# Abolfazlmsl/Oriented-Object-Detection

Measured on AMD Instinct MI355X. Metric: 416px tiles/sec (whole node), YOLOv11n-OBB 3ch, higher is better.
Workload: dtype f32; 1 GPU; YOLOv11n-OBB 3ch 416x416 tiled inference, single-scale (BASELINE configs[1]): forward + decode + ProbIoU NMS + border filter + per-tile merge + final polygon-IoU merge; step_pipelining=True, nc=12, weights=synthetic seeded, cls bias -8 (no checkpoint offline), final_detections=12170

## Files before the change

oriented-object-detection_amd/csrc/c3k2f32.h:

```cpp
#pragma once
#include <hip/hip_runtime.h>

#include <vector>

#include "conv.h"

namespace obb {

struct C3k2F32Launch {
    TensorRef cat;
    TensorRef out;
    const float *w1 = nullptr, *w2 = nullptr, *wc = nullptr;
    const float *b1 = nullptr, *b2 = nullptr, *bc = nullptr;
    int B = 0, H = 0, W = 0, C = 16, CO = 64;
};

bool c3k2f32_supported(int C, int CO, int H, int W);
std::vector<int> c3k2f32_cout_perm(int CO);
void c3k2f32_tile(int H, int W, int &TH, int &TW);
hipError_t launch_c3k2f32(const C3k2F32Launch &L, hipStream_t st);

}
```

oriented-object-detection_amd/csrc/c3k2f32.hip:

```cpp
#include "c3k2f32.h"

#include <algorithm>
#include <mutex>

namespace obb {

typedef __attribute__((ext_vector_type(4))) float f32x4;
typedef __attribute__((ext_vector_type(4))) unsigned int u32x4;

struct C3k2Params {
    const float *cat; int64_t cat_bs; int cat_cs, cat_co; unsigned cat_span;
    float *out; int64_t out_bs; int out_cs, out_co, out_blk, out_ps;
    const float *wall, *b1, *b2;
    int H, W, TH, TW, tiles_x, tiles_y;
    float inv_xw, inv_tw2, inv_tw;
};

__device__ __forceinline__ float silu32c(float x) { return x * __builtin_amdgcn_rcpf(1.0f + __expf(-x)); }

constexpr int kC3MaxX = 448, kC3MaxT = 324;

template <int C, int CO>
__global__ __launch_bounds__(512, 4) void k_c3k2_f32(const C3k2Params P) {
    extern __shared__ __attribute__((aligned(16))) char smem[];
    constexpr int NT = 512, CH = C / 2, PSTX = C * 4 + 16, PSTT = CH * 4 + 16;
    constexpr int CPK1 = C / 4, KP1 = 9 * CPK1 / 4, CPK2 = CH / 4, KP2 = (9 * CPK2) / 4, KR2 = (9 * CPK2) % 4, KPC = 3 * C / 16, NFC = CO / 16;
    static_assert((9 * CPK1) % 4 == 0, "conv 1: whole pieces only");
    constexpr int XOFF = 0, TOFF = kC3MaxX * PSTX, W1OFF = TOFF + kC3MaxT * PSTT, W2OFF = W1OFF + KP1 * 1024, WCOFF = W2OFF + KP2 * 1024 + KR2 * 256,
                  BCOFF = WCOFF + NFC * KPC * 1024, NWCH = (BCOFF + CO * 4 - W1OFF) / 16;
    constexpr int F1 = 3, F2 = 2;
    constexpr unsigned NOPIX = 0xffffffffu;
    const int tid = threadIdx.x, lane = tid & 63, wave = __builtin_amdgcn_readfirstlane(tid >> 6), g = lane >> 4, pl = lane & 15;
    const int t = blockIdx.x, tx_i = t % P.tiles_x, r_ = t / P.tiles_x, ty_i = r_ % P.tiles_y, b = r_ / P.tiles_y;
    const int oy0 = ty_i * P.TH, ox0 = tx_i * P.TW;
    const int XW = P.TW + 4, XH = P.TH + 4, TW2 = P.TW + 2, TH2 = P.TH + 2;
    const int npix1 = TH2 * TW2, npix2 = P.TH * P.TW;

    const __amdgpu_buffer_rsrc_t cat_rsrc = __builtin_amdgcn_make_buffer_rsrc((void *)(P.cat + (int64_t)b * P.cat_bs + P.cat_co), 0, (int)P.cat_span, 0x00020000);
    const __amdgpu_buffer_rsrc_t w_rsrc = __builtin_amdgcn_make_buffer_rsrc((void *)P.wall, 0, NWCH * 16, 0x00020000);
    constexpr int MAXLD = (kC3MaxX * CPK1 + NT - 1) / NT, MAXW = (NWCH + NT - 1) / NT;
    u32x4 xr[MAXLD], wr[MAXW];
    const int nchunkX = XH * XW * CPK1;
#pragma unroll
    for (int k = 0; k < MAXLD; ++k) {
        const int idx = tid + k * NT, pix = idx / CPK1, c = idx - pix * CPK1;
        const int iy = (int)(((float)pix + 0.5f) * P.inv_xw), ix = pix - iy * XW;
        const int gy = oy0 - 2 + iy, gx = ox0 - 2 + ix;
        const bool ok = idx < nchunkX && gy >= 0 && gy < P.H && gx >= 0 && gx < P.W;
        xr[k] = __builtin_amdgcn_raw_buffer_load_b128(cat_rsrc, ok ? (unsigned)((((int64_t)gy * P.W + gx) * P.cat_cs + C + c * 4) * 4) : NOPIX, 0, 0);
    }
#pragma unroll
    for (int k = 0; k < MAXW; ++k) wr[k] = __builtin_amdgcn_raw_buffer_load_b128(w_rsrc, (unsigned)min(tid + k * NT, NWCH - 1) * 16u, 0, 0);
    const int nfrag1 = (npix1 + 15) >> 4, nfrag2 = (npix2 + 15) >> 4;
    f32x4 y0v[F2];
    int opix[F2];
    int xc[F2], tb[F2];
#pragma unroll
    for (int i = 0; i < F2; ++i) {
        const int p0 = (wave + 8 * i) * 16 + pl, p = min(p0, npix2 - 1);
        const int r = (int)(((float)p + 0.5f) * P.inv_tw), x = p - r * P.TW;
        const int oy = oy0 + r, ox = ox0 + x;
        const bool ok = p0 < npix2 && oy < P.H && ox < P.W;
        opix[i] = ok ? oy * P.W + ox : -1;
        y0v[i] = __builtin_bit_cast(f32x4, __builtin_amdgcn_raw_buffer_load_b128(cat_rsrc, ok ? (unsigned)(((int64_t)opix[i] * P.cat_cs + g * 4) * 4) : NOPIX, 0, 0));
        xc[i] = ((r + 2) * XW + x + 2) * PSTX;
        tb[i] = (r * TW2 + x) * PSTT;
    }
#pragma unroll
    for (int k = 0; k < MAXLD; ++k) {
        const int idx = tid + k * NT, pix = idx / CPK1, c = idx - pix * CPK1;
        if (idx < nchunkX) *reinterpret_cast<u32x4 *>(smem + XOFF + pix * PSTX + c * 16) = xr[k];
    }
#pragma unroll
    for (int k = 0; k < MAXW; ++k) {
        const int idx = tid + k * NT;
        if (idx < NWCH) *reinterpret_cast<u32x4 *>(smem + W1OFF + idx * 16) = wr[k];
    }
    __syncthreads();

    {
        int xb[F1];
        bool val[F1];
#pragma unroll
        for (int i = 0; i < F1; ++i) {
            const int f = wave + 8 * i;
            val[i] = f < nfrag1;
            const int p = min(f * 16 + pl, npix1 - 1);
            const int r = (int)(((float)p + 0.5f) * P.inv_tw2), x = p - r * TW2;
            xb[i] = (r * XW + x) * PSTX;
        }
        f32x4 acc[F1];
#pragma unroll
        for (int i = 0; i < F1; ++i) acc[i] = f32x4{0.f, 0.f, 0.f, 0.f};
        for (int piece = 0; piece < KP1; ++piece) {
            const f32x4 w = *reinterpret_cast<const f32x4 *>(smem + W1OFF + piece * 1024 + lane * 16);
            const int q = piece * 4 + g, tap = q / CPK1, c0 = q - tap * CPK1, dy = (tap * 11) >> 5, dx = tap - dy * 3;
            const int off = (dy * XW + dx) * PSTX + c0 * 16;
            f32x4 a[F1];
#pragma unroll
            for (int i = 0; i < F1; ++i) a[i] = *reinterpret_cast<const f32x4 *>(smem + XOFF + xb[i] + off);
#pragma unroll
            for (int s = 0; s < 4; ++s)
#pragma unroll
                for (int i = 0; i < F1; ++i)
                    if (val[i]) acc[i] = __builtin_amdgcn_mfma_f32_16x16x4f32(w[s], a[i][s], acc[i], 0, 0, 0);
        }
        const float4 bv = *reinterpret_cast<const float4 *>(P.b1 + 4 * g);
#pragma unroll
        for (int i = 0; i < F1; ++i) {
            const int p = (wave + 8 * i) * 16 + pl;
            if (!val[i] || p >= npix1 || 4 * g >= CH) continue;
            const int r = (int)(((float)p + 0.5f) * P.inv_tw2), x = p - r * TW2;
            const int gy = oy0 - 1 + r, gx = ox0 - 1 + x;
            const bool inside = gy >= 0 && gy < P.H && gx >= 0 && gx < P.W;
            float4 o = make_float4(0.f, 0.f, 0.f, 0.f);
            if (inside) o = make_float4(silu32c(acc[i][0] + bv.x), silu32c(acc[i][1] + bv.y), silu32c(acc[i][2] + bv.z), silu32c(acc[i][3] + bv.w));
            *reinterpret_cast<float4 *>(smem + TOFF + (r * TW2 + x) * PSTT + g * 16) = o;
        }
    }
    __syncthreads();

    bool val2[F2];
#pragma unroll
    for (int i = 0; i < F2; ++i) val2[i] = wave + 8 * i < nfrag2;
    f32x4 acc2[F2];
#pragma unroll
    for (int i = 0; i < F2; ++i) acc2[i] = f32x4{0.f, 0.f, 0.f, 0.f};
#pragma unroll
    for (int piece = 0; piece < KP2; ++piece) {
        const f32x4 w = *reinterpret_cast<const f32x4 *>(smem + W2OFF + piece * 1024 + lane * 16);
        const int q = piece * 4 + g, tap = q / CPK2, c0 = q - tap * CPK2, dy = (tap * 11) >> 5, dx = tap - dy * 3;
        const int off = (dy * TW2 + dx) * PSTT + c0 * 16;
        f32x4 a[F2];
#pragma unroll
        for (int i = 0; i < F2; ++i) a[i] = *reinterpret_cast<const f32x4 *>(smem + TOFF + tb[i] + off);
#pragma unroll
        for (int s = 0; s < 4; ++s)
#pragma unroll
            for (int i = 0; i < F2; ++i)
                if (val2[i]) acc2[i] = __builtin_amdgcn_mfma_f32_16x16x4f32(w[s], a[i][s], acc2[i], 0, 0, 0);
    }
#pragma unroll
    for (int rr = 0; rr < KR2; ++rr) {
        const float w1 = *reinterpret_cast<const float *>(smem + W2OFF + KP2 * 1024 + rr * 256 + lane * 4);
        const int q = KP2 * 4 + rr, tap = q / CPK2, c0 = q - tap * CPK2, dy = (tap * 11) >> 5, dx = tap - dy * 3;
        const int off = (dy * TW2 + dx) * PSTT + c0 * 16 + g * 4;
#pragma unroll
        for (int i = 0; i < F2; ++i) {
            const float a1 = *reinterpret_cast<const float *>(smem + TOFF + tb[i] + off);
            if (val2[i]) acc2[i] = __builtin_amdgcn_mfma_f32_16x16x4f32(w1, a1, acc2[i], 0, 0, 0);
        }
    }
    f32x4 y1v[F2], y2v[F2];
    {
        const float4 bv = *reinterpret_cast<const float4 *>(P.b2 + 4 * g);
#pragma unroll
        for (int i = 0; i < F2; ++i) {
            y1v[i] = *reinterpret_cast<const f32x4 *>(smem + XOFF + xc[i] + g * 16);
            y2v[i][0] = y1v[i][0] + silu32c(acc2[i][0] + bv.x); y2v[i][1] = y1v[i][1] + silu32c(acc2[i][1] + bv.y);
            y2v[i][2] = y1v[i][2] + silu32c(acc2[i][2] + bv.z); y2v[i][3] = y1v[i][3] + silu32c(acc2[i][3] + bv.w);
        }
    }

    f32x4 acc3[F2][NFC];
#pragma unroll
    for (int i = 0; i < F2; ++i)
#pragma unroll
        for (int nf = 0; nf < NFC; ++nf) acc3[i][nf] = f32x4{0.f, 0.f, 0.f, 0.f};
#pragma unroll
    for (int piece = 0; piece < KPC; ++piece) {
        f32x4 bop[F2];
#pragma unroll
        for (int i = 0; i < F2; ++i) bop[i] = piece == 0 ? y0v[i] : (piece == 1 ? y1v[i] : y2v[i]);
#pragma unroll
        for (int nf = 0; nf < NFC; ++nf) {
            const f32x4 w = *reinterpret_cast<const f32x4 *>(smem + WCOFF + (nf * KPC + piece) * 1024 + lane * 16);
#pragma unroll
            for (int s = 0; s < 4; ++s)
#pragma unroll
                for (int i = 0; i < F2; ++i)
                    if (val2[i]) acc3[i][nf] = __builtin_amdgcn_mfma_f32_16x16x4f32(w[s], bop[i][s], acc3[i][nf], 0, 0, 0);
        }
    }
#pragma unroll
    for (int i = 0; i < F2; ++i) {
        if (!val2[i] || opix[i] < 0) continue;
        const int ca = P.out_co + 16 * g;
        float *op = P.out + (int64_t)b * P.out_bs + (int64_t)opix[i] * P.out_cs + (P.out_blk ? (int64_t)(ca >> 3) * P.out_ps + (ca & 7) : (int64_t)ca);
#pragma unroll
        for (int nf = 0; nf < NFC; ++nf) {
            const float4 bv = *reinterpret_cast<const float4 *>(smem + BCOFF + (nf * 16 + 4 * g) * 4);
            const float4 o = make_float4(silu32c(acc3[i][nf][0] + bv.x), silu32c(acc3[i][nf][1] + bv.y), silu32c(acc3[i][nf][2] + bv.z), silu32c(acc3[i][nf][3] + bv.w));
            float *o4 = P.out_blk ? op + (int64_t)(nf >> 1) * P.out_ps + 4 * (nf & 1) : op + 4 * nf;
            *reinterpret_cast<float4 *>(o4) = o;
        }
    }
}

void c3k2f32_tile(int H, int W, int &TH, int &TW) {
    TW = std::min(W, 52);
    if (W > 52 && W % 52 && W % 2 == 0 && W / 2 <= 52) TW = W / 2;
    int th = 1;
    while (th + 1 <= H && (th + 5) * (TW + 4) <= kC3MaxX && (th + 3) * (TW + 2) <= kC3MaxT && (th + 3) * (TW + 2) <= 24 * 16 && (th + 1) * TW <= 16 * 16) ++th;
    TH = th;
}

bool c3k2f32_supported(int C, int CO, int H, int W) {
    if (C != 16 || CO != 64 || H < 1 || W < 1) return false;
    int TH, TW;
    c3k2f32_tile(H, W, TH, TW);
    return (TH + 4) * (TW + 4) <= kC3MaxX && (TH + 2) * (TW + 2) <= kC3MaxT && (TH + 2) * (TW + 2) <= 24 * 16 && TH * TW <= 16 * 16;
}

std::vector<int> c3k2f32_cout_perm(int CO) {
    std::vector<int> p(CO);
    for (int f = 0; f < CO / 16; ++f)
        for (int r = 0; r < 16; ++r) p[16 * f + r] = 16 * (r >> 2) + 4 * f + (r & 3);
    return p;
}

hipError_t launch_c3k2f32(const C3k2F32Launch &L, hipStream_t st) {
    if (!c3k2f32_supported(L.C, L.CO, L.H, L.W) || L.cat.cpb || (L.cat.cs & 3) || (L.cat.co & 3) || !L.w1 || !L.b1 || !L.b2 || L.B < 1) return hipErrorInvalidValue;
    if (L.out.cpb && !(L.out.cpb == 2 && L.out.cs == 8 && L.out.co % 8 == 0 && L.out.ps > 0)) return hipErrorInvalidValue;
    if (!L.out.cpb && ((L.out.cs | L.out.co) & 3)) return hipErrorInvalidValue;
    C3k2Params P;
    P.cat = (const float *)L.cat.p; P.cat_bs = L.cat.bs; P.cat_cs = L.cat.cs; P.cat_co = L.cat.co;
    const int64_t span = ((int64_t)L.H * L.W * L.cat.cs - L.cat.co) * 4;
    if (span <= 0 || span >= (1ll << 32) - 65536) return hipErrorInvalidValue;
    P.cat_span = (unsigned)span;
    P.out = (float *)L.out.p; P.out_bs = L.out.bs; P.out_cs = L.out.cs; P.out_co = L.out.co; P.out_blk = L.out.cpb ? 1 : 0; P.out_ps = (int)L.out.ps;
    P.wall = L.w1; P.b1 = L.b1; P.b2 = L.b2;
    P.H = L.H; P.W = L.W;
    c3k2f32_tile(L.H, L.W, P.TH, P.TW);
    P.tiles_x = (L.W + P.TW - 1) / P.TW; P.tiles_y = (L.H + P.TH - 1) / P.TH;
    P.inv_xw = 1.0f / (float)(P.TW + 4); P.inv_tw2 = 1.0f / (float)(P.TW + 2); P.inv_tw = 1.0f / (float)P.TW;
    const int64_t ntiles = (int64_t)L.B * P.tiles_y * P.tiles_x;
    if (ntiles >= (1ll << 31)) return hipErrorInvalidValue;
    constexpr int C = 16, CO = 64;
    constexpr size_t lds = (size_t)kC3MaxX * (C * 4 + 16) + (size_t)kC3MaxT * (C / 2 * 4 + 16) + 9 * 1024 + (4 * 1024 + 2 * 256) + (CO / 16) * 3 * 1024 + CO * 4;
    static std::once_flag once;
    static hipError_t attr_err = hipSuccess;
    std::call_once(once, [] { attr_err = hipFuncSetAttribute((const void *)k_c3k2_f32<16, 64>, hipFuncAttributeMaxDynamicSharedMemorySize, 80 * 1024); });
    if (attr_err != hipSuccess) return attr_err;
    hipLaunchKernelGGL((k_c3k2_f32<16, 64>), dim3((unsigned)ntiles), dim3(512), lds, st, P);
    return hipGetLastError();
}

}
```

oriented-object-detection_amd/csrc/engine.hip:

```cpp
#include <algorithm>
#include <cmath>
#include <cstdlib>
#include <cstring>
#include <map>
#include <memory>
#include <string>
#include <tuple>

#include "bneck.h"
#include "c3k2f32.h"
#include "c3kimg.h"
#include "ctx.h"
#include "dwpw.h"
#include "f32path.h"
#include "front.h"
#include "nnops.h"
#include "pw32.h"
#include "stem.h"

namespace obb {

static constexpr int kRegMax = 16;

struct ConvRecord {
// ... 551 lines not shown
            st.second.assign(a->b, a->b + a->c2);
            st.second.insert(st.second.end(), b->b, b->b + b->c2);
            ConvRecord r = *a;
            r.name = nm; r.c2 = a->c2 + b->c2; r.w = st.first.data(); r.b = st.second.data();
            M.recs[nm] = r;
        }
        return nm;
    }

    bool bottleneck(const std::string &name, Slice in, int H, int W, Slice out, double e, const char *cv2name = nullptr, Slice y0 = Slice(),
                    Slice cv2out = Slice()) {
        int c_ = (int)(out.C * e);
        if (M.bneck && in.buf >= 0 && in.buf == out.buf && P.bufs[in.buf].blk == in.C && in.C == out.C && c_ * 2 == in.C &&
            bneck_supported(in.C, H, W)) {
            const ConvRecord *r1 = rec(name + ".cv1"), *r2 = rec(name + ".cv2");
            if (!r1 || !r2 || err) return false;
            if (r1->k == 3 && r2->k == 3 && r1->s == 1 && r2->s == 1 && r1->g == 1 && r2->g == 1 && r1->act && r2->act && r1->c1 == in.C &&
                r1->c2 == c_ && r2->c1 == c_ && r2->c2 == in.C) {
                Op op;
                op.type = OP_BNECK; op.name = name; op.in = in; op.out = out; op.H = H; op.W = W; op.Ho = H; op.Wo = W;
                BneckLaunch &L = op.bneck;
                L.H = H; L.W = W; L.C = in.C; L.f16 = M.f16;
                ConvTiling t1{1, 1, 1, 1, in.C}, t2{1, 1, 1, in.C / 16, c_};
                L.w1pk = upload(pack_conv_weights(r1->w, c_, in.C, 3, t1, nullptr, 0, M.f16));
                L.w2pk = upload(pack_conv_weights(r2->w, in.C, c_, 3, t2, nullptr, 0, M.f16));
                std::vector<float> b1(128, 0.f), b2(128, 0.f);
                for (int c = 0; c < c_; ++c) b1[c] = r1->b[c];
                for (int c = 0; c < in.C; ++c) b2[c] = r2->b[c];
                L.bias1 = upload(b1); L.bias2 = upload(b2);
                op.macs = (double)H * W * 9.0 * in.C * c_ * 2;
                bool fused_cv2 = false;
                const ConvRecord *rc = cv2name ? rec(cv2name) : nullptr;
                if (rc && M.o.bneck_cv2 && rc->k == 1 && rc->s == 1 && rc->g == 1 && rc->act && rc->c1 == 3 * in.C && rc->c2 == cv2out.C && cv2out.buf >= 0 &&
                    !P.bufs[cv2out.buf].virt && y0.buf == in.buf && y0.C == in.C && y0.co + in.C == in.co && in.co + in.C == out.co &&
                    bneck_cv2_supported(in.C, rc->c2)) {
                    ConvTiling tc{1, 1, 1, rc->c2 / 16, in.C == 32 ? 96 : 32};
                    L.CO = rc->c2;
                    L.wc32pk = upload(pack_conv_weights(rc->w, rc->c2, rc->c1, 1, tc, nullptr, 0, M.f16));
                    if (in.C == 16) L.wc16pk = upload(pack_bneck_k16(rc->w, rc->c2, rc->c1, 32, M.f16));
                    std::vector<float> bc(128 + 64, 0.f);
                    for (int c = 0; c < rc->c2; ++c) bc[c] = rc->b[c];
                    L.biasc = upload(bc);
                    op.name = name + "+" + cv2name;
                    op.out = cv2out; op.res = y0;
                    op.macs += (double)H * W * rc->c1 * rc->c2;
                    fused_cv2 = true;
                }
                P.macs_per_img += op.macs;
                P.ops.push_back(op);
                if (fused_cv2) P.named[cv2name] = cv2out;
                else P.named[name + ".cv2"] = out;
                return fused_cv2;
            }
        }
        int t = buf(H, W, c_, name + ".t");
        conv(name + ".cv1", in, H, W, whole(t));
        conv(name + ".cv2", whole(t), H, W, out, in);
        return false;
    }

    void c3k(const std::string &name, Slice in, int H, int W, Slice out, int n) {
        int c_ = out.C / 2;
        const bool img_on = M.hmerge && M.o.c3kimg && !M.f32;
        if (img_on && in.buf >= 0 && out.buf >= 0 && !P.bufs[in.buf].blk && !P.bufs[in.buf].virt && !P.bufs[out.buf].blk &&
            c3kimg_supported(H, W, in.C, c_, out.C, n)) {
            const std::string names[6] = {name + ".cv1", name + ".cv2", name + ".m.0.cv1", name + ".m.0.cv2", name + ".m.1.cv1", name + ".m.1.cv2"};
            const ConvRecord *r[7];
            bool ok = true;
            for (int i = 0; i < 6; ++i) { r[i] = rec(names[i]); ok = ok && r[i]; }
            r[6] = rec(name + ".cv3"); ok = ok && r[6];
            if (!ok || err) return;
            auto is = [](const ConvRecord *q, int k, int c1, int c2) { return q->k == k && q->s == 1 && q->g == 1 && q->act && q->c1 == c1 && q->c2 == c2; };
            if (is(r[0], 1, in.C, c_) && is(r[1], 1, in.C, c_) && is(r[2], 3, c_, c_) && is(r[3], 3, c_, c_) && is(r[4], 3, c_, c_) && is(r[5], 3, c_, c_) &&
                is(r[6], 1, 2 * c_, out.C)) {
                std::vector<bf16_t> stream;
                std::vector<float> bias(6 * 128, 0.f);
                auto add = [&](const float *w, int cout, int cin, int ks) {
                    ConvTiling t{1, 1, 1, 4, cin};
                    std::vector<bf16_t> pk = pack_conv_weights(w, cout, cin, ks, t, nullptr, 0, M.f16);
                    stream.insert(stream.end(), pk.begin(), pk.end());
                };
                std::vector<float> w01((size_t)2 * c_ * in.C);
                std::copy(r[0]->w, r[0]->w + (size_t)c_ * in.C, w01.begin());
                std::copy(r[1]->w, r[1]->w + (size_t)c_ * in.C, w01.begin() + (size_t)c_ * in.C);
                add(w01.data(), 2 * c_, in.C, 1);
                for (int c = 0; c < c_; ++c) { bias[c] = r[0]->b[c]; bias[c_ + c] = r[1]->b[c]; }
                for (int i = 2; i < 6; ++i) {
                    add(r[i]->w, c_, c_, 3);
                    for (int c = 0; c < c_; ++c) bias[(i - 1) * 128 + c] = r[i]->b[c];
                }
                add(r[6]->w, out.C, 2 * c_, 1);
                for (int c = 0; c < out.C; ++c) bias[5 * 128 + c] = r[6]->b[c];
                if ((int)(stream.size() / 8) != c3kimg_pieces()) { err = set_error(ctx, OBB_ERR_STATE, "c3k image kernel: weight stream has %zu pieces", stream.size() / 8); return; }
                Op op;
                op.type = OP_C3KIMG; op.name = name; op.in = in; op.out = out; op.H = H; op.W = W; op.Ho = H; op.Wo = W;
                op.c3kimg.wts = upload(stream); op.c3kimg.bias = upload(bias); op.c3kimg.f16 = M.f16;
                op.macs = (double)H * W * ((double)in.C * 2 * c_ + 4.0 * 9 * c_ * c_ + 2.0 * c_ * out.C);
                P.macs_per_img += op.macs;
                P.ops.push_back(op);
                P.named[name + ".cv3"] = out;
                return;
            }
        }
        const std::string mn = n >= 2 ? merged_record(name + ".cv1", name + ".cv2") : std::string();
        if (!mn.empty()) {
            int ab = buf(H, W, 2 * c_, name + ".cat", false, c_);
            conv(mn, in, H, W, whole(ab));
            P.named[name + ".cv1"] = sub(ab, 0, c_);
            Slice cur = sub(ab, 0, c_);
            for (int i = 0; i < n; ++i) {
                Slice dst = (i == n - 1) ? sub(ab, 0, c_) : whole(buf(H, W, c_, name + ".m" + std::to_string(i)));
                bottleneck(name + ".m." + std::to_string(i), cur, H, W, dst, 1.0);
                cur = dst;
            }
            P.named[name + ".cv2"] = sub(ab, c_, c_);
            conv(name + ".cv3", whole(ab), H, W, out);
            return;
        }
        if (err) return;
        int cat = buf(H, W, 2 * c_, name + ".cat");
        int a = buf(H, W, c_, name + ".a");
        conv(name + ".cv1", in, H, W, whole(a));
        Slice cur = whole(a);
        for (int i = 0; i < n; ++i) {
            Slice dst = (i == n - 1) ? sub(cat, 0, c_) : whole(buf(H, W, c_, name + ".m" + std::to_string(i)));
            bottleneck(name + ".m." + std::to_string(i), cur, H, W, dst, 1.0);
            cur = dst;
        }
        conv(name + ".cv2", in, H, W, sub(cat, c_, c_));
        conv(name + ".cv3", whole(cat), H, W, out);
    }

    void c3k2(int li, Slice in, int H, int W, Slice out, int n, bool use_c3k, double e, const char *prod = nullptr, Slice pin = Slice(), int pH = 0,
              int pW = 0) {
        std::string name = "model." + std::to_string(li);
        int c = (int)(out.C * e);
        if (prod) {
            int cat = buf(H, W, (2 + n) * c, name + ".cat", false, use_c3k ? 0 : c);
            conv(prod, pin, pH, pW, sub(cat, 0, 2 * c), Slice(), -1, nullptr, (name + ".cv1").c_str());
            c3k2_rest(name, cat, c, H, W, out, n, use_c3k);
            return;
        }
        int cat = buf(H, W, (2 + n) * c, name + ".cat", false, use_c3k ? 0 : c);
        conv(name + ".cv1", in, H, W, sub(cat, 0, 2 * c));
        c3k2_rest(name, cat, c, H, W, out, n, use_c3k);
    }
    bool c3k2_f32(const std::string &name, int cat, int c, int H, int W, Slice out) {
        if (!M.f32 || !M.tail || !M.o.c3k2f || out.buf < 0 || P.bufs[out.buf].virt || P.bufs[cat].blk32 || !c3k2f32_supported(c, out.C, H, W)) return false;
        const ConvRecord *r1 = rec(name + ".m.0.cv1"), *r2 = rec(name + ".m.0.cv2"), *rc = rec(name + ".cv2");
        if (!r1 || !r2 || !rc || err) return false;
        auto is = [](const ConvRecord *q, int k, int c1, int c2) { return q->k == k && q->s == 1 && q->g == 1 && q->act && q->c1 == c1 && q->c2 == c2; };
        if (!is(r1, 3, c, c / 2) || !is(r2, 3, c / 2, c) || !is(rc, 1, 3 * c, out.C)) return false;
        const std::vector<int> perm = c3k2f32_cout_perm(out.C);
        const Conv32Tiling t1{1, 1, c, 1, 1, 1, 1}, t2{1, 1, c / 2, 1, 1, 1, 1}, tc{1, 1, 3 * c, out.C / 16, 1, 1, 1};
        std::vector<float> wall = pack_conv32_weights(r1->w, c / 2, c, 3, t1, nullptr, false);
        const std::vector<float> w2 = pack_conv32_weights(r2->w, c, c / 2, 3, t2, nullptr, false), wc = pack_conv32_weights(rc->w, out.C, 3 * c, 1, tc, perm.data(), false);
        wall.insert(wall.end(), w2.begin(), w2.end());
        wall.insert(wall.end(), wc.begin(), wc.end());
        for (int i = 0; i < out.C; ++i) wall.push_back(rc->b[perm[i]]);
        if (wall.size() != (size_t)(9 * 256 + 4 * 256 + 2 * 64 + (out.C / 16) * 3 * 256 + out.C)) { err = set_error(ctx, OBB_ERR_STATE, "c3k2 fp32 kernel: weight image has %zu floats", wall.size()); return false; }
        std::vector<float> b1(64, 0.f), b2(64, 0.f);
        for (int i = 0; i < c / 2; ++i) b1[i] = r1->b[i];
        for (int i = 0; i < c; ++i) b2[i] = r2->b[i];
        Op op;
        op.type = OP_C3K2F32; op.name = name + ".m.0+" + name + ".cv2"; op.in = sub(cat, 0, 2 * c); op.out = out; op.H = H; op.W = W; op.Ho = H; op.Wo = W;
        C3k2F32Launch &L = op.c3k2f;
        L.H = H; L.W = W; L.C = c; L.CO = out.C;
        L.w1 = upload(wall); L.b1 = upload(b1); L.b2 = upload(b2);
        op.macs = (double)H * W * (9.0 * c * (c / 2) * 2 + 3.0 * c * out.C);
        P.macs_per_img += op.macs;
        P.ops.push_back(op);
        P.named[name + ".cv2"] = out;
        return true;
    }

    void c3k2_rest(const std::string &name, int cat, int c, int H, int W, Slice out, int n, bool use_c3k) {
        if (n == 1 && !use_c3k && c3k2_f32(name, cat, c, H, W, out)) return;
        if (n == 1 && !use_c3k && bottleneck(name + ".m.0", sub(cat, c, c), H, W, sub(cat, 2 * c, c), 0.5, (name + ".cv2").c_str(), sub(cat, 0, c), out)) return;
        if (n == 1 && !use_c3k) { conv(name + ".cv2", whole(cat), H, W, out); return; }
        for (int i = 0; i < n; ++i) {
            Slice src = sub(cat, (1 + i) * c, c), dst = sub(cat, (2 + i) * c, c);
            if (use_c3k) c3k(name + ".m." + std::to_string(i), src, H, W, dst, 2);
            else bottleneck(name + ".m." + std::to_string(i), src, H, W, dst, 0.5);
        }
        conv(name + ".cv2", whole(cat), H, W, out);
    }


    int build() {
        const int h = P.h, w = P.w;
        const bool big = M.scale == "m" || M.scale == "l" || M.scale == "x";
        const int n2 = reps(2);
        const int c64 = ch(64), c128 = ch(128), c256 = ch(256), c512 = ch(512), c1024 = ch(1024);
        const int H2 = h / 2, W2 = w / 2, H4 = h / 4, W4 = w / 4, H8 = h / 8, W8 = w / 8, H16 = h / 16, W16 = w / 16, H32 = h / 32, W32 = w / 32;
        const bool fold = M.upfold && c1024 % 64 == 0 && c512 % 64 == 0 && c1024 + c512 >= 128 && !big;
        int cat13 = -1, cat16 = -1;
        if (!fold) {
            cat13 = buf(H16, W16, c1024 + c512, "cat13");
            cat16 = buf(H8, W8, c512 + c512, "cat16");
        }
        int cat19 = buf(H16, W16, c256 + c512, "cat19");
        int cat22 = buf(H32, W32, c512 + c1024, "cat22");
        Slice x4 = fold ? whole(buf(H8, W8, c512, "x4", false, 0, true)) : sub(cat16, c512, c512), x6 = fold ? whole(buf(H16, W16, c512, "x6", false, 0, true)) : sub(cat13, c1024, c512);
        Slice x10 = sub(cat22, c512, c1024), x13 = sub(cat19, c256, c512);

        const bool t1 = tail16_ok("model.1", "model.2.cv1", H2, W2), t3 = tail16_ok("model.3", "model.4.cv1", H4, W4);
        use_front = t1 && front_ok(h, w);
        int b0 = use_front ? -1 : buf(H2, W2, c64, "x0");
        if (!use_front) conv("model.0", Slice{-1, 0, M.ch}, h, w, whole(b0));
        int b1 = t1 ? -1 : buf(H4, W4, c128, "x1");
        if (!t1) conv("model.1", whole(b0), H2, W2, whole(b1));
        int b2 = buf(H4, W4, c256, "x2", false, 16, true);
        if (t1) c3k2(2, Slice(), H4, W4, whole(b2), n2, big, 0.25, "model.1", use_front ? Slice{-1, 0, c64} : whole(b0), H2, W2);
        else c3k2(2, whole(b1), H4, W4, whole(b2), n2, big, 0.25);
        int b3 = t3 ? -1 : buf(H8, W8, c256, "x3");
        if (!t3) conv("model.3", whole(b2), H4, W4, whole(b3));
        if (t3) c3k2(4, Slice(), H8, W8, x4, n2, big, 0.25, "model.3", whole(b2), H4, W4);
        else c3k2(4, whole(b3), H8, W8, x4, n2, big, 0.25);
        int b5 = buf(H16, W16, c512, "x5");
        conv("model.5", x4, H8, W8, whole(b5));
        c3k2(6, whole(b5), H16, W16, x6, n2, true, 0.5);
        int b7 = buf(H32, W32, c1024, "x7");
        conv("model.7", x6, H16, W16, whole(b7));
        int b8 = buf(H32, W32, c1024, "x8");
        c3k2(8, whole(b7), H32, W32, whole(b8), n2, true, 0.5);
        int c_ = c1024 / 2;
        int cat9 = buf(H32, W32, 4 * c_, "cat9");
        conv("model.9.cv1", whole(b8), H32, W32, sub(cat9, 0, c_));
        if (M.o.sppf_fuse && c_ % 32 == 0 && (size_t)H32 * W32 * (M.f32 ? 256 : 128) <= 64 * 1024) {
            Op op; op.type = OP_SPPF; op.name = "sppf.pools"; op.in = sub(cat9, 0, c_); op.out = whole(cat9); op.H = H32; op.W = W32; op.Ho = H32; op.Wo = W32;
            P.ops.push_back(op);
        } else {
            for (int i = 0; i < 3; ++i) pool(sub(cat9, i * c_, c_), H32, W32, sub(cat9, (i + 1) * c_, c_));
        }
        int b9 = buf(H32, W32, c1024, "x9");
        conv("model.9.cv2", whole(cat9), H32, W32, whole(b9));
        int cp = c1024 / 2, nh = cp / 64, hd = cp / nh, kd = hd / 2;
        int t10 = buf(H32, W32, 2 * cp, "psa.ab");
        conv("model.10.cv1", whole(b9), H32, W32, whole(t10));
        Slice bsl = sub(t10, cp, cp);
        int qkvb = buf(H32, W32, cp + 2 * nh * kd, "psa.qkv"), ao = buf(H32, W32, cp, "psa.attn"), po = buf(H32, W32, cp, "psa.pe"),
            ff = buf(H32, W32, 2 * cp, "psa.ffn");
        std::vector<int> perm(cp + 2 * nh * kd);
        for (int hh = 0; hh < nh; ++hh) {
            int src0 = hh * (2 * kd + hd);
            for (int d = 0; d < kd; ++d) { perm[hh * kd + d] = src0 + d; perm[nh * kd + hh * kd + d] = src0 + kd + d; }
            for (int d = 0; d < hd; ++d) perm[2 * nh * kd + hh * hd + d] = src0 + 2 * kd + d;
        }
        for (int i = 0; i < n2; ++i) {
            std::string nm = "model.10.m." + std::to_string(i);
            conv(nm + ".attn.qkv", bsl, H32, W32, whole(qkvb), Slice(), -1, perm.data());
            Op at; at.type = OP_ATTN; at.name = nm + ".attn"; at.in = whole(qkvb); at.out = whole(ao); at.H = H32; at.W = W32; at.Ho = H32; at.Wo = W32;
            at.N = H32 * W32; at.nh = nh; at.kd = kd; at.hd = hd;
            P.macs_per_img += (double)nh * ((double)at.N * at.N * kd + (double)at.N * at.N * hd);
            P.ops.push_back(at);
            P.named[nm + ".attn"] = whole(ao);
            dwconv(nm + ".attn.pe", sub(qkvb, 2 * nh * kd, cp), H32, W32, whole(po), whole(ao));
            conv(nm + ".attn.proj", whole(po), H32, W32, bsl, bsl);
            conv(nm + ".ffn.0", bsl, H32, W32, whole(ff));
            conv(nm + ".ffn.1", whole(ff), H32, W32, bsl, bsl);
        }
        conv("model.10.cv2", whole(t10), H32, W32, x10);
        if (fold) cat13 = vbuf(H16, W16, x10, x6, "cat13");
        else upsample(x10, H32, W32, sub(cat13, 0, c1024));
        c3k2(13, whole(cat13), H16, W16, x13, n2, big, 0.5);
        if (fold) cat16 = vbuf(H8, W8, x13, x4, "cat16");
        else upsample(x13, H16, W16, sub(cat16, 0, c512));
        auto feat_blk = [&](int C, int H, int W) { return M.f32 && M.tail && M.o.dwpw && plan_dwpw32(C, std::max(c256, std::min(M.nc, 100)), H, W).TH > 0; };
        int b16 = buf(H8, W8, c256, "x16", false, 0, feat_blk(c256, H8, W8));
        c3k2(16, whole(cat16), H8, W8, whole(b16), n2, big, 0.5);
        P.ops.back().signal_feat = 0;
        conv("model.17", whole(b16), H8, W8, sub(cat19, 0, c256));
        int b19 = buf(H16, W16, c512, "x19", false, 0, feat_blk(c512, H16, W16));
        c3k2(19, whole(cat19), H16, W16, whole(b19), n2, big, 0.5);
        P.ops.back().signal_feat = 1;
        conv("model.20", whole(b19), H16, W16, sub(cat22, 0, c512));
        int b22 = buf(H32, W32, c1024, "x22");
        c3k2(22, whole(cat22), H32, W32, whole(b22), n2, true, 0.5);
        P.ops.back().signal_feat = 2;
        const int chs[3] = {c256, c512, c1024};
        const int feats[3] = {b16, b19, b22};
        const int Hs[3] = {H8, H16, H32}, Ws[3] = {W8, W16, W32};
        int c2 = std::max(std::max(16, chs[0] / 4), kRegMax * 4), c3 = std::max(chs[0], std::min(M.nc, 100)), c4 = std::max(chs[0] / 4, 1);
        P.no = 4 * kRegMax + M.nc + 1;
        P.no_pad = (P.no + 3) / 4 * 4;
        int off = 0;
        for (int i = 0; i < 3; ++i) { P.lvl_off[i] = off; off += Hs[i] * Ws[i]; }
        P.A = off;
        auto mark_branch = [&](size_t first, int lane, int level) { (void)first; (void)lane; (void)level; };
        Slice u1s[3];
        for (int i = 0; i < 3; ++i) {
            size_t first_op = P.ops.size();
            std::string p = "model.23.cv2." + std::to_string(i), p4 = "model.23.cv4." + std::to_string(i);
            const bool pair80 = M.o.pair && !M.f32 && P.bufs[feats[i]].C == 64 && c2 == 64 && c4 == 16 && Hs[i] % 13 == 0 && Ws[i] % 13 == 0;
            const std::string mn = (!M.f32 && c2 % 16 == 0 && c4 % 16 == 0 && (Hs[i] * Ws[i] <= 256 || pair80)) ? merged_record(p + ".0", p4 + ".0") : std::string();
            if (err) return err;
            int t1, t2 = buf(Hs[i], Ws[i], c2, p + ".t2");
            if (!mn.empty()) {
                int hb = buf(Hs[i], Ws[i], c2 + c4, p + ".t1u1", false, pair80 ? 0 : 16);
                conv(mn, whole(feats[i]), Hs[i], Ws[i], whole(hb));
                P.named[p + ".0"] = sub(hb, 0, c2);
                P.named[p4 + ".0"] = sub(hb, c2, c4);
                u1s[i] = sub(hb, c2, c4);
                Slice t1s = sub(hb, 0, c2);
                if (tail_ok(p + ".1", p + ".2", Hs[i], Ws[i])) {
                    conv(p + ".1", t1s, Hs[i], Ws[i], Slice{-2, 0, 4 * kRegMax}, Slice(), i, nullptr, (p + ".2").c_str());
                } else {
                    conv(p + ".1", t1s, Hs[i], Ws[i], whole(t2));
                    conv(p + ".2", whole(t2), Hs[i], Ws[i], Slice{-2, 0, 4 * kRegMax}, Slice(), i);
                }
                mark_branch(first_op, 1, i);
                continue;
            }
// ... 589 lines not shown
```

Before: 32520 tiles/s.

## Pack two pixels per MFMA row in the c3k2 first conv to fill idle output rows

The first 3x3 conv in the fused fp32 C3k2 kernel has only C/2=8 output channels, so half of each 16-row MFMA output sat idle. The weights are now repacked so one MFMA computes two adjacent pixels times eight couts, walking four tap columns per kernel row, which halves the fragment count. Each wave now dispatches on a compile-time fragment count of one or two instead of predicating every MFMA, and phase 2 assigns waves in reverse order to balance load. The cost is 12 weight pieces instead of 9, slightly more LDS, and more intricate indexing, with a per-device attribute cache added at launch.

```diff
diff --git a/oriented-object-detection_amd/csrc/c3k2f32.h b/oriented-object-detection_amd/csrc/c3k2f32.h
--- a/oriented-object-detection_amd/csrc/c3k2f32.h
+++ b/oriented-object-detection_amd/csrc/c3k2f32.h
@@ -17,6 +17,7 @@
 
 bool c3k2f32_supported(int C, int CO, int H, int W);
 std::vector<int> c3k2f32_cout_perm(int CO);
+std::vector<float> c3k2f32_pack_w1(const float *w_oihw, int C);
 void c3k2f32_tile(int H, int W, int &TH, int &TW);
 hipError_t launch_c3k2f32(const C3k2F32Launch &L, hipStream_t st);
 
diff --git a/oriented-object-detection_amd/csrc/c3k2f32.hip b/oriented-object-detection_amd/csrc/c3k2f32.hip
--- a/oriented-object-detection_amd/csrc/c3k2f32.hip
+++ b/oriented-object-detection_amd/csrc/c3k2f32.hip
@@ -1,7 +1,9 @@
 #include "c3k2f32.h"
 
 #include <algorithm>
+#include <map>
 #include <mutex>
+#include <type_traits>
 
 namespace obb {
 
@@ -13,7 +15,7 @@
     float *out; int64_t out_bs; int out_cs, out_co, out_blk, out_ps;
     const float *wall, *b1, *b2;
     int H, W, TH, TW, tiles_x, tiles_y;
-    float inv_xw, inv_tw2, inv_tw;
+    float inv_xw, inv_pw, inv_tw;
 };
 
 __device__ __forceinline__ float silu32c(float x) { return x * __builtin_amdgcn_rcpf(1.0f + __expf(-x)); }
@@ -24,17 +26,18 @@
 __global__ __launch_bounds__(512, 4) void k_c3k2_f32(const C3k2Params P) {
     extern __shared__ __attribute__((aligned(16))) char smem[];
     constexpr int NT = 512, CH = C / 2, PSTX = C * 4 + 16, PSTT = CH * 4 + 16;
-    constexpr int CPK1 = C / 4, KP1 = 9 * CPK1 / 4, CPK2 = CH / 4, KP2 = (9 * CPK2) / 4, KR2 = (9 * CPK2) % 4, KPC = 3 * C / 16, NFC = CO / 16;
-    static_assert((9 * CPK1) % 4 == 0, "conv 1: whole pieces only");
+    constexpr int CPK1 = C / 4, KP1 = 12, CPK2 = CH / 4, KP2 = (9 * CPK2) / 4, KR2 = (9 * CPK2) % 4, KPC = 3 * C / 16, NFC = CO / 16;
+    static_assert(CPK1 == 4 && 2 * CH == 16, "conv 1: one piece = one tap column of a pixel pair (4 chunks), two pixels x C/2 couts = 16 rows");
     constexpr int XOFF = 0, TOFF = kC3MaxX * PSTX, W1OFF = TOFF + kC3MaxT * PSTT, W2OFF = W1OFF + KP1 * 1024, WCOFF = W2OFF + KP2 * 1024 + KR2 * 256,
                   BCOFF = WCOFF + NFC * KPC * 1024, NWCH = (BCOFF + CO * 4 - W1OFF) / 16;
-    constexpr int F1 = 3, F2 = 2;
+    constexpr int NWV = NT / 64, F1 = 2, F2 = 2;
     constexpr unsigned NOPIX = 0xffffffffu;
     const int tid = threadIdx.x, lane = tid & 63, wave = __builtin_amdgcn_readfirstlane(tid >> 6), g = lane >> 4, pl = lane & 15;
     const int t = blockIdx.x, tx_i = t % P.tiles_x, r_ = t / P.tiles_x, ty_i = r_ % P.tiles_y, b = r_ / P.tiles_y;
     const int oy0 = ty_i * P.TH, ox0 = tx_i * P.TW;
-    const int XW = P.TW + 4, XH = P.TH + 4, TW2 = P.TW + 2, TH2 = P.TH + 2;
-    const int npix1 = TH2 * TW2, npix2 = P.TH * P.TW;
+    const int XW = P.TW + 4, XH = P.TH + 4, TW2 = P.TW + 2, TH2 = P.TH + 2, PW = (TW2 + 1) >> 1;
+    const int npair1 = TH2 * PW, npix2 = P.TH * P.TW;
+    const int wv2 = NWV - 1 - wave;
 
     const __amdgpu_buffer_rsrc_t cat_rsrc = __builtin_amdgcn_make_buffer_rsrc((void *)(P.cat + (int64_t)b * P.cat_bs + P.cat_co), 0, (int)P.cat_span, 0x00020000);
     const __amdgpu_buffer_rsrc_t w_rsrc = __builtin_amdgcn_make_buffer_rsrc((void *)P.wall, 0, NWCH * 16, 0x00020000);
@@ -51,13 +54,13 @@
     }
 #pragma unroll
     for (int k = 0; k < MAXW; ++k) wr[k] = __builtin_amdgcn_raw_buffer_load_b128(w_rsrc, (unsigned)min(tid + k * NT, NWCH - 1) * 16u, 0, 0);
-    const int nfrag1 = (npix1 + 15) >> 4, nfrag2 = (npix2 + 15) >> 4;
+    const int nfrag1 = (npair1 + 15) >> 4, nfrag2 = (npix2 + 15) >> 4;
     f32x4 y0v[F2];
     int opix[F2];
     int xc[F2], tb[F2];
 #pragma unroll
     for (int i = 0; i < F2; ++i) {
-        const int p0 = (wave + 8 * i) * 16 + pl, p = min(p0, npix2 - 1);
+        const int p0 = (wv2 + NWV * i) * 16 + pl, p = min(p0, npix2 - 1);
         const int r = (int)(((float)p + 0.5f) * P.inv_tw), x = p - r * P.TW;
         const int oy = oy0 + r, ox = ox0 + x;
         const bool ok = p0 < npix2 && oy < P.H && ox < P.W;
@@ -78,123 +81,127 @@
     }
     __syncthreads();
 
-    {
-        int xb[F1];
-        bool val[F1];
-#pragma unroll
-        for (int i = 0; i < F1; ++i) {
-            const int f = wave + 8 * i;
-            val[i] = f < nfrag1;
-            const int p = min(f * 16 + pl, npix1 - 1);
-            const int r = (int)(((float)p + 0.5f) * P.inv_tw2), x = p - r * TW2;
-            xb[i] = (r * XW + x) * PSTX;
-        }
-        f32x4 acc[F1];
-#pragma unroll
-        for (int i = 0; i < F1; ++i) acc[i] = f32x4{0.f, 0.f, 0.f, 0.f};
-        for (int piece = 0; piece < KP1; ++piece) {
-            const f32x4 w = *reinterpret_cast<const f32x4 *>(smem + W1OFF + piece * 1024 + lane * 16);
-            const int q = piece * 4 + g, tap = q / CPK1, c0 = q - tap * CPK1, dy = (tap * 11) >> 5, dx = tap - dy * 3;
-            const int off = (dy * XW + dx) * PSTX + c0 * 16;
-            f32x4 a[F1];
-#pragma unroll
-            for (int i = 0; i < F1; ++i) a[i] = *reinterpret_cast<const f32x4 *>(smem + XOFF + xb[i] + off);
-#pragma unroll
-            for (int s = 0; s < 4; ++s)
-#pragma unroll
-                for (int i = 0; i < F1; ++i)
-                    if (val[i]) acc[i] = __builtin_amdgcn_mfma_f32_16x16x4f32(w[s], a[i][s], acc[i], 0, 0, 0);
-        }
-        const float4 bv = *reinterpret_cast<const float4 *>(P.b1 + 4 * g);
-#pragma unroll
-        for (int i = 0; i < F1; ++i) {
-            const int p = (wave + 8 * i) * 16 + pl;
-            if (!val[i] || p >= npix1 || 4 * g >= CH) continue;
-            const int r = (int)(((float)p + 0.5f) * P.inv_tw2), x = p - r * TW2;
+    static_assert(F1 == 2 && F2 == 2, "the dispatch below knows one or two fragments per wave");
+
+    auto conv1 = [&](auto nf_) {
+        constexpr int NF = decltype(nf_)::value;
+        int xb[NF], xb3[NF];
+#pragma unroll
+        for (int i = 0; i < NF; ++i) {
+            const int p = min((wave + NWV * i) * 16 + pl, npair1 - 1);
+            const int r = (int)(((float)p + 0.5f) * P.inv_pw), xe = (p - r * PW) * 2;
+            xb[i] = (r * XW + xe) * PSTX + g * 16;
+            xb3[i] = xb[i] + min(3, XW - 1 - xe) * PSTX;
+        }
+        f32x4 acc[NF];
+#pragma unroll
+        for (int i = 0; i < NF; ++i) acc[i] = f32x4{0.f, 0.f, 0.f, 0.f};
+#pragma unroll
+        for (int dy = 0; dy < 3; ++dy)
+#pragma unroll
+            for (int dxp = 0; dxp < 4; ++dxp) {
+                const f32x4 w = *reinterpret_cast<const f32x4 *>(smem + W1OFF + (dy * 4 + dxp) * 1024 + lane * 16);
+                f32x4 a[NF];
+#pragma unroll
+                for (int i = 0; i < NF; ++i) a[i] = *reinterpret_cast<const f32x4 *>(smem + XOFF + (dxp < 3 ? xb[i] + dxp * PSTX : xb3[i]) + dy * XW * PSTX);
+#pragma unroll
+                for (int s = 0; s < 4; ++s)
+#pragma unroll
+                    for (int i = 0; i < NF; ++i) acc[i] = __builtin_amdgcn_mfma_f32_16x16x4f32(w[s], a[i][s], acc[i], 0, 0, 0);
+            }
+        const float4 bv = *reinterpret_cast<const float4 *>(P.b1 + 4 * (g & 1));
+#pragma unroll
+        for (int i = 0; i < NF; ++i) {
+            const int p = (wave + NWV * i) * 16 + pl;
+            if (p >= npair1) continue;
+            const int r = (int)(((float)p + 0.5f) * P.inv_pw), x = (p - r * PW) * 2 + (g >> 1);
+            if (x >= TW2) continue;
             const int gy = oy0 - 1 + r, gx = ox0 - 1 + x;
             const bool inside = gy >= 0 && gy < P.H && gx >= 0 && gx < P.W;
             float4 o = make_float4(0.f, 0.f, 0.f, 0.f);
             if (inside) o = make_float4(silu32c(acc[i][0] + bv.x), silu32c(acc[i][1] + bv.y), silu32c(acc[i][2] + bv.z), silu32c(acc[i][3] + bv.w));
-            *reinterpret_cast<float4 *>(smem + TOFF + (r * TW2 + x) * PSTT + g * 16) = o;
-        }
-    }
+            *reinterpret_cast<float4 *>(smem + TOFF + (r * TW2 + x) * PSTT + (g & 1) * 16) = o;
+        }
+    };
+    if (wave + NWV < nfrag1) conv1(std::integral_constant<int, 2>{});
+    else if (wave < nfrag1) conv1(std::integral_constant<int, 1>{});
     __syncthreads();
 
-    bool val2[F2];
-#pragma unroll
-    for (int i = 0; i < F2; ++i) val2[i] = wave + 8 * i < nfrag2;
-    f32x4 acc2[F2];
-#pragma unroll
-    for (int i = 0; i < F2; ++i) acc2[i] = f32x4{0.f, 0.f, 0.f, 0.f};
-#pragma unroll
-    for (int piece = 0; piece < KP2; ++piece) {
-        const f32x4 w = *reinterpret_cast<const f32x4 *>(smem + W2OFF + piece * 1024 + lane * 16);
-        const int q = piece * 4 + g, tap = q / CPK2, c0 = q - tap * CPK2, dy = (tap * 11) >> 5, dx = tap - dy * 3;
-        const int off = (dy * TW2 + dx) * PSTT + c0 * 16;
-        f32x4 a[F2];
-#pragma unroll
-        for (int i = 0; i < F2; ++i) a[i] = *reinterpret_cast<const f32x4 *>(smem + TOFF + tb[i] + off);
-#pragma unroll
-        for (int s = 0; s < 4; ++s)
-#pragma unroll
-            for (int i = 0; i < F2; ++i)
-                if (val2[i]) acc2[i] = __builtin_amdgcn_mfma_f32_16x16x4f32(w[s], a[i][s], acc2[i], 0, 0, 0);
-    }
-#pragma unroll
-    for (int rr = 0; rr < KR2; ++rr) {
-        const float w1 = *reinterpret_cast<const float *>(smem + W2OFF + KP2 * 1024 + rr * 256 + lane * 4);
-        const int q = KP2 * 4 + rr, tap = q / CPK2, c0 = q - tap * CPK2, dy = (tap * 11) >> 5, dx = tap - dy * 3;
-        const int off = (dy * TW2 + dx) * PSTT + c0 * 16 + g * 4;
-#pragma unroll
-        for (int i = 0; i < F2; ++i) {
-            const float a1 = *reinterpret_cast<const float *>(smem + TOFF + tb[i] + off);
-            if (val2[i]) acc2[i] = __builtin_amdgcn_mfma_f32_16x16x4f32(w1, a1, acc2[i], 0, 0, 0);
-        }
-    }
-    f32x4 y1v[F2], y2v[F2];
-    {
-        const float4 bv = *reinterpret_cast<const float4 *>(P.b2 + 4 * g);
-#pragma unroll
-        for (int i = 0; i < F2; ++i) {
-            y1v[i] = *reinterpret_cast<const f32x4 *>(smem + XOFF + xc[i] + g * 16);
-            y2v[i][0] = y1v[i][0] + silu32c(acc2[i][0] + bv.x); y2v[i][1] = y1v[i][1] + silu32c(acc2[i][1] + bv.y);
-            y2v[i][2] = y1v[i][2] + silu32c(acc2[i][2] + bv.z); y2v[i][3] = y1v[i][3] + silu32c(acc2[i][3] + bv.w);
-        }
-    }
-
-    f32x4 acc3[F2][NFC];
-#pragma unroll
-    for (int i = 0; i < F2; ++i)
-#pragma unroll
-        for (int nf = 0; nf < NFC; ++nf) acc3[i][nf] = f32x4{0.f, 0.f, 0.f, 0.f};
-#pragma unroll
-    for (int piece = 0; piece < KPC; ++piece) {
-        f32x4 bop[F2];
-#pragma unroll
-        for (int i = 0; i < F2; ++i) bop[i] = piece == 0 ? y0v[i] : (piece == 1 ? y1v[i] : y2v[i]);
-#pragma unroll
-        for (int nf = 0; nf < NFC; ++nf) {
-            const f32x4 w = *reinterpret_cast<const f32x4 *>(smem + WCOFF + (nf * KPC + piece) * 1024 + lane * 16);
+    auto phase2 = [&](auto nf_) {
+        constexpr int NF = decltype(nf_)::value;
+        f32x4 acc2[NF];
+#pragma unroll
+        for (int i = 0; i < NF; ++i) acc2[i] = f32x4{0.f, 0.f, 0.f, 0.f};
+#pragma unroll
+        for (int piece = 0; piece < KP2; ++piece) {
+            const f32x4 w = *reinterpret_cast<const f32x4 *>(smem + W2OFF + piece * 1024 + lane * 16);
+            const int q = piece * 4 + g, tap = q / CPK2, c0 = q - tap * CPK2, dy = (tap * 11) >> 5, dx = tap - dy * 3;
+            const int off = (dy * TW2 + dx) * PSTT + c0 * 16;
+            f32x4 a[NF];
+#pragma unroll
+            for (int i = 0; i < NF; ++i) a[i] = *reinterpret_cast<const f32x4 *>(smem + TOFF + tb[i] + off);
 #pragma unroll
             for (int s = 0; s < 4; ++s)
 #pragma unroll
-                for (int i = 0; i < F2; ++i)
-                    if (val2[i]) acc3[i][nf] = __builtin_amdgcn_mfma_f32_16x16x4f32(w[s], bop[i][s], acc3[i][nf], 0, 0, 0);
-        }
-    }
-#pragma unroll
-    for (int i = 0; i < F2; ++i) {
-        if (!val2[i] || opix[i] < 0) continue;
-        const int ca = P.out_co + 16 * g;
-        float *op = P.out + (int64_t)b * P.out_bs + (int64_t)opix[i] * P.out_cs + (P.out_blk ? (int64_t)(ca >> 3) * P.out_ps + (ca & 7) : (int64_t)ca);
-#pragma unroll
-        for (int nf = 0; nf < NFC; ++nf) {
-            const float4 bv = *reinterpret_cast<const float4 *>(smem + BCOFF + (nf * 16 + 4 * g) * 4);
-            const float4 o = make_float4(silu32c(acc3[i][nf][0] + bv.x), silu32c(acc3[i][nf][1] + bv.y), silu32c(acc3[i][nf][2] + bv.z), silu32c(acc3[i][nf][3] + bv.w));
-            float *o4 = P.out_blk ? op + (int64_t)(nf >> 1) * P.out_ps + 4 * (nf & 1) : op + 4 * nf;
-            *reinterpret_cast<float4 *>(o4) = o;
-        }
-    }
+                for (int i = 0; i < NF; ++i) acc2[i] = __builtin_amdgcn_mfma_f32_16x16x4f32(w[s], a[i][s], acc2[i], 0, 0, 0);
+        }
+#pragma unroll
+        for (int rr = 0; rr < KR2; ++rr) {
+            const float w1 = *reinterpret_cast<const float *>(smem + W2OFF + KP2 * 1024 + rr * 256 + lane * 4);
+            const int q = KP2 * 4 + rr, tap = q / CPK2, c0 = q - tap * CPK2, dy = (tap * 11) >> 5, dx = tap - dy * 3;
+            const int off = (dy * TW2 + dx) * PSTT + c0 * 16 + g * 4;
+#pragma unroll
+            for (int i = 0; i < NF; ++i) {
+                const float a1 = *reinterpret_cast<const float *>(smem + TOFF + tb[i] + off);
+                acc2[i] = __builtin_amdgcn_mfma_f32_16x16x4f32(w1, a1, acc2[i], 0, 0, 0);
+            }
+        }
+        f32x4 y1v[NF], y2v[NF];
+        {
+            const float4 bv = *reinterpret_cast<const float4 *>(P.b2 + 4 * g);
+#pragma unroll
+            for (int i = 0; i < NF; ++i) {
+                y1v[i] = *reinterpret_cast<const f32x4 *>(smem + XOFF + xc[i] + g * 16);
+                y2v[i][0] = y1v[i][0] + silu32c(acc2[i][0] + bv.x); y2v[i][1] = y1v[i][1] + silu32c(acc2[i][1] + bv.y);
+                y2v[i][2] = y1v[i][2] + silu32c(acc2[i][2] + bv.z); y2v[i][3] = y1v[i][3] + silu32c(acc2[i][3] + bv.w);
+            }
+        }
+
+        f32x4 acc3[NF][NFC];
+#pragma unroll
+        for (int i = 0; i < NF; ++i)
+#pragma unroll
+            for (int nf = 0; nf < NFC; ++nf) acc3[i][nf] = f32x4{0.f, 0.f, 0.f, 0.f};
+#pragma unroll
+        for (int piece = 0; piece < KPC; ++piece) {
+            f32x4 bop[NF];
+#pragma unroll
+            for (int i = 0; i < NF; ++i) bop[i] = piece == 0 ? y0v[i] : (piece == 1 ? y1v[i] : y2v[i]);
+#pragma unroll
+            for (int nf = 0; nf < NFC; ++nf) {
+                const f32x4 w = *reinterpret_cast<const f32x4 *>(smem + WCOFF + (nf * KPC + piece) * 1024 + lane * 16);
+#pragma unroll
+                for (int s = 0; s < 4; ++s)
+#pragma unroll
+                    for (int i = 0; i < NF; ++i) acc3[i][nf] = __builtin_amdgcn_mfma_f32_16x16x4f32(w[s], bop[i][s], acc3[i][nf], 0, 0, 0);
+            }
+        }
+#pragma unroll
+        for (int i = 0; i < NF; ++i) {
+            if (opix[i] < 0) continue;
+            const int ca = P.out_co + 16 * g;
+            float *op = P.out + (int64_t)b * P.out_bs + (int64_t)opix[i] * P.out_cs + (P.out_blk ? (int64_t)(ca >> 3) * P.out_ps + (ca & 7) : (int64_t)ca);
+#pragma unroll
+            for (int nf = 0; nf < NFC; ++nf) {
+                const float4 bv = *reinterpret_cast<const float4 *>(smem + BCOFF + (nf * 16 + 4 * g) * 4);
+                const float4 o = make_float4(silu32c(acc3[i][nf][0] + bv.x), silu32c(acc3[i][nf][1] + bv.y), silu32c(acc3[i][nf][2] + bv.z), silu32c(acc3[i][nf][3] + bv.w));
+                float *o4 = P.out_blk ? op + (int64_t)(nf >> 1) * P.out_ps + 4 * (nf & 1) : op + 4 * nf;
+                *reinterpret_cast<float4 *>(o4) = o;
+            }
+        }
+    };
+    if (wv2 + NWV < nfrag2) phase2(std::integral_constant<int, 2>{});
+    else if (wv2 < nfrag2) phase2(std::integral_constant<int, 1>{});
 }
 
 void c3k2f32_tile(int H, int W, int &TH, int &TW) {
@@ -209,7 +216,7 @@
     if (C != 16 || CO != 64 || H < 1 || W < 1) return false;
     int TH, TW;
     c3k2f32_tile(H, W, TH, TW);
-    return (TH + 4) * (TW + 4) <= kC3MaxX && (TH + 2) * (TW + 2) <= kC3MaxT && (TH + 2) * (TW + 2) <= 24 * 16 && TH * TW <= 16 * 16;
+    return (TH + 4) * (TW + 4) <= kC3MaxX && (TH + 2) * (TW + 2) <= kC3MaxT && (TH + 2) * ((TW + 3) / 2) <= 16 * 16 && TH * TW <= 16 * 16;
 }
 
 std::vector<int> c3k2f32_cout_perm(int CO) {
@@ -217,6 +224,19 @@
     for (int f = 0; f < CO / 16; ++f)
         for (int r = 0; r < 16; ++r) p[16 * f + r] = 16 * (r >> 2) + 4 * f + (r & 3);
     return p;
+}
+
+std::vector<float> c3k2f32_pack_w1(const float *w, int C) {
+    const int CH = C / 2;
+    std::vector<float> out((size_t)12 * 256, 0.f);
+    for (int dy = 0; dy < 3; ++dy)
+        for (int dxp = 0; dxp < 4; ++dxp)
+            for (int lane = 0; lane < 64; ++lane)
+                for (int s = 0; s < 4; ++s) {
+                    const int row = lane & 15, c = (lane >> 4) * 4 + s, co = row % CH, dx = dxp - row / CH;
+                    if (dx >= 0 && dx < 3) out[((size_t)(dy * 4 + dxp) * 64 + lane) * 4 + s] = w[((size_t)co * C + c) * 9 + dy * 3 + dx];
+                }
+    return out;
 }
 
 hipError_t launch_c3k2f32(const C3k2F32Launch &L, hipStream_t st) {
@@ -233,15 +253,24 @@
     P.H = L.H; P.W = L.W;
     c3k2f32_tile(L.H, L.W, P.TH, P.TW);
     P.tiles_x = (L.W + P.TW - 1) / P.TW; P.tiles_y = (L.H + P.TH - 1) / P.TH;
-    P.inv_xw = 1.0f / (float)(P.TW + 4); P.inv_tw2 = 1.0f / (float)(P.TW + 2); P.inv_tw = 1.0f / (float)P.TW;
+    P.inv_xw = 1.0f / (float)(P.TW + 4); P.inv_pw = 1.0f / (float)((P.TW + 3) / 2); P.inv_tw = 1.0f / (float)P.TW;
     const int64_t ntiles = (int64_t)L.B * P.tiles_y * P.tiles_x;
     if (ntiles >= (1ll << 31)) return hipErrorInvalidValue;
     constexpr int C = 16, CO = 64;
-    constexpr size_t lds = (size_t)kC3MaxX * (C * 4 + 16) + (size_t)kC3MaxT * (C / 2 * 4 + 16) + 9 * 1024 + (4 * 1024 + 2 * 256) + (CO / 16) * 3 * 1024 + CO * 4;
-    static std::once_flag once;
-    static hipError_t attr_err = hipSuccess;
-    std::call_once(once, [] { attr_err = hipFuncSetAttribute((const void *)k_c3k2_f32<16, 64>, hipFuncAttributeMaxDynamicSharedMemorySize, 80 * 1024); });
-    if (attr_err != hipSuccess) return attr_err;
+    constexpr size_t lds = (size_t)kC3MaxX * (C * 4 + 16) + (size_t)kC3MaxT * (C / 2 * 4 + 16) + 12 * 1024 + (4 * 1024 + 2 * 256) + (CO / 16) * 3 * 1024 + CO * 4;
+    static_assert(lds <= 80 * 1024, "two workgroups per CU");
+    static std::mutex mu;
+    static std::map<int, bool> attr_set;
+    int dev = 0;
+    hipError_t e = hipGetDevice(&dev);
+    if (e != hipSuccess) return e;
+    {
+        std::lock_guard<std::mutex> lock(mu);
+        if (!attr_set.count(dev)) {
+            if ((e = hipFuncSetAttribute((const void *)k_c3k2_f32<16, 64>, hipFuncAttributeMaxDynamicSharedMemorySize, 80 * 1024)) != hipSuccess) return e;
+            attr_set[dev] = true;
+        }
+    }
     hipLaunchKernelGGL((k_c3k2_f32<16, 64>), dim3((unsigned)ntiles), dim3(512), lds, st, P);
     return hipGetLastError();
 }
diff --git a/oriented-object-detection_amd/csrc/engine.hip b/oriented-object-detection_amd/csrc/engine.hip
--- a/oriented-object-detection_amd/csrc/engine.hip
+++ b/oriented-object-detection_amd/csrc/engine.hip
@@ -727,13 +727,13 @@
         auto is = [](const ConvRecord *q, int k, int c1, int c2) { return q->k == k && q->s == 1 && q->g == 1 && q->act && q->c1 == c1 && q->c2 == c2; };
         if (!is(r1, 3, c, c / 2) || !is(r2, 3, c / 2, c) || !is(rc, 1, 3 * c, out.C)) return false;
         const std::vector<int> perm = c3k2f32_cout_perm(out.C);
-        const Conv32Tiling t1{1, 1, c, 1, 1, 1, 1}, t2{1, 1, c / 2, 1, 1, 1, 1}, tc{1, 1, 3 * c, out.C / 16, 1, 1, 1};
-        std::vector<float> wall = pack_conv32_weights(r1->w, c / 2, c, 3, t1, nullptr, false);
+        const Conv32Tiling t2{1, 1, c / 2, 1, 1, 1, 1}, tc{1, 1, 3 * c, out.C / 16, 1, 1, 1};
+        std::vector<float> wall = c3k2f32_pack_w1(r1->w, c);
         const std::vector<float> w2 = pack_conv32_weights(r2->w, c, c / 2, 3, t2, nullptr, false), wc = pack_conv32_weights(rc->w, out.C, 3 * c, 1, tc, perm.data(), false);
         wall.insert(wall.end(), w2.begin(), w2.end());
         wall.insert(wall.end(), wc.begin(), wc.end());
         for (int i = 0; i < out.C; ++i) wall.push_back(rc->b[perm[i]]);
-        if (wall.size() != (size_t)(9 * 256 + 4 * 256 + 2 * 64 + (out.C / 16) * 3 * 256 + out.C)) { err = set_error(ctx, OBB_ERR_STATE, "c3k2 fp32 kernel: weight image has %zu floats", wall.size()); return false; }
+        if (wall.size() != (size_t)(12 * 256 + 4 * 256 + 2 * 64 + (out.C / 16) * 3 * 256 + out.C)) { err = set_error(ctx, OBB_ERR_STATE, "c3k2 fp32 kernel: weight image has %zu floats", wall.size()); return false; }
         std::vector<float> b1(64, 0.f), b2(64, 0.f);
         for (int i = 0; i < c / 2; ++i) b1[i] = r1->b[i];
         for (int i = 0; i < c; ++i) b2[i] = r2->b[i];
```

New measurement: 32830 tiles/s, median of 6. No clear change (+0.9%).
